# tataganesh/Query-Efficient-Approx-to-improve-OCR

Measured on AMD Instinct MI355X. Metric: patch-images/sec UNet->CRNN->CTC fwd+bwd, 32x128 grey, higher is better.
Workload: dtype f32 (GEMMs as scaled 2 x fp16 split products — three fp16 MFMAs per fp32 multiply-add — fp32 accumulate); 1 GPU; BASELINE configs[2]: full minibatch step of train_nn_area.py:212-287 — Phase A (UNet eval fwd, TopKCER k = 5 % of the minibatch, inner_limit = 4 jitter replicas fused in the batch dim, CRNN train-BN fwd+bwd, Adam(CRNN)) + Phase B (UNet train-BN -> CRNN BN-eval -> CTC mean + MSE -> backward -> Adam(UNet)) + greedy decode -> CER -> update_cer (:290-304) on synthetic POS-style 32x128 patches; batch_per_gpu=2048, global_batch=2048, full_step=True, crnn_wgrad=True, parallelism=dp1, hipgraph=False

## Files before the change

### query-efficient-approx-to-improve-ocr_amd/csrc/conv_wgrad.hip

```cpp
#include "common.h"
#include <type_traits>

namespace {

struct WgArgs {
  const float* p;
  const float* q;
  float* out;
  int B, PH, PW, QH, QW, R, C, KH, KW, pad_h, pad_w, stride_h, stride_w, ldp, ldq;
  int M, chunk, splits, accumulate;
  int r_tiles, c_tiles, tiles;
  long long slab;
  const float* pmax;
  const float* qmax;
};

constexpr int BKP_MAX = 32;

template <int P_LD, int Q_LD, int BKP>
struct WgGather {
  static constexpr int TPR = 256 / BKP;
  int grow, gl;
  int g_img, g_ph, g_pw;
  int qhw, dr, er, eq;
// ... 799 lines not shown
        *reinterpret_cast<bf16x4*>(Ps + 2 * P_PLANE + o) = l;
      }
    }
#pragma unroll
    for (int i = 0; i < NQ; ++i) {
      const int e = tid + 256 * i;
      const int c4 = e % CC4, hq = e / CC4;
      if (hq < HP) {
        const int o = row_off(hq, c4, CB);
        if constexpr (F16) {
          f16x4 h, l;
          qea_split2_f16(qreg[i], sq, h, l);
          *reinterpret_cast<f16x4*>(Qs + o) = h;
          *reinterpret_cast<f16x4*>(Qs + Q_PLANE + o) = l;
        } else {
          bf16x4 h, m, l;
          qea_split3(qreg[i], h, m, l);
          *reinterpret_cast<bf16x4*>(Qs + o) = h;
          *reinterpret_cast<bf16x4*>(Qs + Q_PLANE + o) = m;
          *reinterpret_cast<bf16x4*>(Qs + 2 * Q_PLANE + o) = l;
        }
      }
    }
  };
  const int g16 = lane >> 4, tq = (lane & 15) >> 2, tpp = lane & 3;
  const int l_pix = (g16 >> 1) * 8 + tq;
  const int l_ch = (g16 & 1) * 16 + tpp * 4;
  auto frag_p = [&](const __bf16* plane, int pix) -> frag_t {
    return __builtin_bit_cast(frag_t, RB == 64 ? tr_frag(plane + pix * 64 + (((wr ^ (pix >> 1)) & 1) << 5) + l_ch, 64) : tr_frag(plane + pix * 32 + l_ch, 32));
  };
  auto frag_q = [&](const __bf16* plane, int pix) -> frag_t {
    return __builtin_bit_cast(frag_t, CB == 64 ? tr_frag(plane + pix * 64 + (((wc ^ (pix >> 1)) & 1) << 5) + l_ch, 64) : tr_frag(plane + pix * 32 + l_ch, 32));
  };
  auto mma = [&](f32x16& a9, const frag_t* af, const frag_t* bf) {
    if constexpr (F16) {
      a9 = __builtin_amdgcn_mfma_f32_32x32x16_f16(af[1], bf[0], a9, 0, 0, 0);
      a9 = __builtin_amdgcn_mfma_f32_32x32x16_f16(af[0], bf[1], a9, 0, 0, 0);
      a9 = __builtin_amdgcn_mfma_f32_32x32x16_f16(af[0], bf[0], a9, 0, 0, 0);
    } else {
      a9 = __builtin_amdgcn_mfma_f32_32x32x16_bf16(af[2], bf[0], a9, 0, 0, 0);
      a9 = __builtin_amdgcn_mfma_f32_32x32x16_bf16(af[0], bf[2], a9, 0, 0, 0);
      a9 = __builtin_amdgcn_mfma_f32_32x32x16_bf16(af[1], bf[1], a9, 0, 0, 0);
      a9 = __builtin_amdgcn_mfma_f32_32x32x16_bf16(af[1], bf[0], a9, 0, 0, 0);
      a9 = __builtin_amdgcn_mfma_f32_32x32x16_bf16(af[0], bf[1], a9, 0, 0, 0);
      a9 = __builtin_amdgcn_mfma_f32_32x32x16_bf16(af[0], bf[0], a9, 0, 0, 0);
    }
  };

  int tile = split;
  if (tile < hp.n_tiles) fetch(tile);
  for (; tile < hp.n_tiles; tile += hp.splits) {
    __syncthreads();
    stage();
    __syncthreads();
    if (tile + hp.splits < hp.n_tiles) fetch(tile + hp.splits);
#pragma unroll 1
    for (int ks = wk; ks < 4; ks += WK) {
      const int py = (ks * 16) / SW, px0 = (ks * 16) % SW;
      frag_t af[NPL];
#pragma unroll
      for (int pl = 0; pl < NPL; ++pl) af[pl] = frag_p(Ps + pl * P_PLANE, ks * 16 + l_pix);
      if constexpr (RB == 32 || F16) {
        auto read_q = [&](int t, frag_t* bfr) {
          const int hq = (py + t / 3) * HW_ + px0 + t % 3 + l_pix;
#pragma unroll
          for (int pl = 0; pl < NPL; ++pl) bfr[pl] = frag_q(Qs + pl * Q_PLANE, hq);
        };
        frag_t bq2[2][NPL];
        read_q(0, bq2[0]);
#pragma unroll
        for (int t = 0; t < 9; ++t) {
          const frag_t* bf = bq2[t & 1];
          if (t + 1 < 9) read_q(t + 1, bq2[(t + 1) & 1]);
          mma(acc[t], af, bf);
          if (t + 1 < 9) {
            __builtin_amdgcn_sched_group_barrier(0x100, 2 * NPL, 0);
            __builtin_amdgcn_sched_group_barrier(0x008, F16 ? 3 : 6, 0);
          }
        }
      } else {
#pragma unroll
        for (int kh = 0; kh < 3; ++kh)
#pragma unroll
          for (int kw = 0; kw < 3; ++kw) {
            const int hq = (py + kh) * HW_ + px0 + kw + l_pix;
            frag_t bf[NPL];
#pragma unroll
            for (int pl = 0; pl < NPL; ++pl) bf[pl] = frag_q(Qs + pl * Q_PLANE, hq);
            mma(acc[kh * 3 + kw], af, bf);
          }
      }
    }
  }
  float* out = ws + ((size_t)split * WK + wk) * R * 9 * C;
  const int fr = lane & 31, fh = lane >> 5;
#pragma unroll
  for (int t = 0; t < 9; ++t)
#pragma unroll
    for (int r = 0; r < 16; ++r) {
      const int rr = r0 + wr * 32 + (r & 3) + 8 * (r >> 2) + 4 * fh;
      out[((size_t)rr * 9 + t) * C + c0 + wc * 32 + fr] = F16 ? (acc[t][r] * inv_p) * inv_q : acc[t][r];
    }
}

__device__ __forceinline__ f16x8 tr_pair128(const char* base) {
  typedef __attribute__((address_space(3))) s16x4* lds_ptr;
  const s16x4 lo = __builtin_amdgcn_ds_read_tr16_b64_v4i16((lds_ptr)(base));
  const s16x4 hi = __builtin_amdgcn_ds_read_tr16_b64_v4i16((lds_ptr)(base + 4 * 128));
  return __builtin_shufflevector(__builtin_bit_cast(f16x4, lo), __builtin_bit_cast(f16x4, hi), 0, 1, 2, 3, 4, 5, 6, 7);
}

__global__ void bias_finalize_kernel(const double* __restrict__ ws, int nblk, int R, float* __restrict__ out, int accumulate) {
  const int c = blockIdx.x * (blockDim.x >> 6) + (threadIdx.x >> 6);
  if (c >= R) return;
  const int lane = threadIdx.x & 63;
  double a = 0;
  for (int k = lane; k < nblk; k += 64) a += ws[(size_t)k * R + c];
  a = qea_wave_sum_d(a);
  if (lane == 0) out[c] = accumulate ? out[c] + (float)a : (float)a;
}

template <int SW>
constexpr size_t halo9_spec_lds() { return (size_t)2 * (2 * 64 * 64 * 2 + 2 * ((64 / SW + 2) * (SW + 2)) * 64 * 2); }

template <int SW>
__global__ __launch_bounds__(512) void wgrad_halo9_spec_kernel(const float* __restrict__ p, const float* __restrict__ q, float* __restrict__ ws, int B,
                                                               int H, int W, int R, int C, int ldp, int ldq, Halo9Plan hp,
                                                               const float* __restrict__ pmax, const float* __restrict__ qmax,
                                                               double* __restrict__ bias_ws) {
  constexpr int TH = 64 / SW, HWD = SW + 2, HH = TH + 2, HP = HH * HWD;
  constexpr int P_PLANE_B = 64 * 64 * 2, Q_PLANE_B = HP * 64 * 2;
  constexpr int BUF_B = 2 * P_PLANE_B + 2 * Q_PLANE_B;
  extern __shared__ __attribute__((aligned(16))) float smem[];
  char* lds = reinterpret_cast<char*>(smem);
  float sp, sq, inv_p, inv_q;
  qea_f16_scale(pmax[0], sp, inv_p);
  qea_f16_scale(qmax[0], sq, inv_q);
  const int tid = threadIdx.x, lane = tid & 63, wave = tid >> 6;
  int bid = qea_xcd_swizzle(blockIdx.x, gridDim.x);
  const int c_blk = bid % hp.c_blks;
  bid /= hp.c_blks;
  const int r_blk = bid % hp.r_blks;
  const int split = bid / hp.r_blks;
  const int r0 = r_blk * 64, c0 = c_blk * 64;
  const int ntl = (hp.n_tiles - split + hp.splits - 1) / hp.splits;

  if (wave >= 4) {
    const int pt = tid - 256;
    constexpr int NP = 64 * 16 / 256, NQ = (HP * 16 + 255) / 256;
    f32x4 preg[NP], qreg[NQ];
    const bool do_bias = bias_ws != nullptr && c_blk == 0;
    double bsum[4] = {0.0, 0.0, 0.0, 0.0};
    auto fetch = [&](int tile) {
      const int tx = tile % hp.tiles_x;
      const int ty = (tile / hp.tiles_x) % hp.tiles_y;
      const int b = tile / (hp.tiles_x * hp.tiles_y);
      const int x0 = tx * SW, y0 = ty * TH;
#pragma unroll
      for (int i = 0; i < NP; ++i) {
        const int e = pt + 256 * i;
        const int c4 = e % 16, pix = e / 16;
        const int py = pix / SW, px = pix - py * SW;
        preg[i] = *reinterpret_cast<const f32x4*>(p + ((size_t)(b * H + y0 + py) * W + x0 + px) * ldp + r0 + c4 * 4);
      }
#pragma unroll
      for (int i = 0; i < NQ; ++i) {
        const int e = pt + 256 * i;
        const int c4 = e % 16, hq = e / 16;
        f32x4 v = {0.f, 0.f, 0.f, 0.f};
        if (hq < HP) {
          const int hy = hq / HWD, hx = hq - hy * HWD;
          const int iy = y0 + hy - 1, ix = x0 + hx - 1;
          if ((unsigned)iy < (unsigned)H && (unsigned)ix < (unsigned)W) v = *reinterpret_cast<const f32x4*>(q + ((size_t)(b * H + iy) * W + ix) * ldq + c0 + c4 * 4);
        }
        qreg[i] = v;
      }
    };
    auto row_off = [](int pix, int c4) { return pix * 64 + ((((c4 >> 3) ^ (pix >> 1)) & 1) << 5) + (c4 & 7) * 4; };
    auto stage = [&](char* buf) {
      _Float16* Ps = reinterpret_cast<_Float16*>(buf);
      _Float16* Qs = reinterpret_cast<_Float16*>(buf + 2 * P_PLANE_B);
#pragma unroll
      for (int i = 0; i < NP; ++i) {
        const int e = pt + 256 * i;
        const int o = row_off(e / 16, e % 16);
        if (do_bias) {
#pragma unroll
          for (int k = 0; k < 4; ++k) bsum[k] += (double)preg[i][k];
        }
        f16x4 h, l;
        qea_split2_f16(preg[i], sp, h, l);
        *reinterpret_cast<f16x4*>(Ps + o) = h;
        *reinterpret_cast<f16x4*>(Ps + P_PLANE_B / 2 + o) = l;
      }
#pragma unroll
      for (int i = 0; i < NQ; ++i) {
        const int e = pt + 256 * i;
        const int hq = e / 16;
        if (hq < HP) {
          const int o = row_off(hq, e % 16);
          f16x4 h, l;
          qea_split2_f16(qreg[i], sq, h, l);
          *reinterpret_cast<f16x4*>(Qs + o) = h;
          *reinterpret_cast<f16x4*>(Qs + Q_PLANE_B / 2 + o) = l;
        }
      }
    };
    if (ntl > 0) {
      fetch(split);
      stage(lds);
      if (ntl > 1) fetch(split + hp.splits);
    }
    __syncthreads();
    for (int t = 0; t < ntl; ++t) {
      if (t + 1 < ntl) stage(lds + ((t + 1) & 1) * BUF_B);
      if (t + 2 < ntl) fetch(split + (t + 2) * hp.splits);
      __syncthreads();
    }
    if (do_bias) {
#pragma unroll
      for (int k = 0; k < 4; ++k) {
        double v = bsum[k];
        v += __shfl_xor(v, 16, 64);
        v += __shfl_xor(v, 32, 64);
        bsum[k] = v;
      }
      if (lane < 16) {
        double* dst = bias_ws + (size_t)(split * 4 + (wave - 4)) * R + r0 + lane * 4;
#pragma unroll
        for (int k = 0; k < 4; ++k) dst[k] = bsum[k];
      }
    }
    return;
  }

  const int wr = wave >> 1, wc = wave & 1;
  f32x16 acc[9];
#pragma unroll
  for (int t = 0; t < 9; ++t)
#pragma unroll
    for (int r = 0; r < 16; ++r) acc[t][r] = 0.f;
  const int g16 = lane >> 4, tq = (lane & 15) >> 2, tpp = lane & 3;
  const int l_pix = (g16 >> 1) * 8 + tq;
  const int l_ch = (g16 & 1) * 16 + tpp * 4;
  const int p_off = l_pix * 128 + ((((wr ^ (l_pix >> 1)) & 1) << 5) + l_ch) * 2;
  int TQ[2][2];
#pragma unroll
  for (int par = 0; par < 2; ++par)
#pragma unroll
    for (int b = 0; b < 2; ++b) {
      const int hs = (par ? (l_pix + 1) >> 1 : l_pix >> 1) + b;
      TQ[par][b] = l_pix * 128 + ((((wc ^ hs) & 1) << 5) + l_ch) * 2;
    }
  __syncthreads();
  for (int t = 0; t < ntl; ++t) {
    const char* buf = lds + (t & 1) * BUF_B;
    const char* Pb = buf + p_off;
    const char* Qb = buf + 2 * P_PLANE_B;
    auto read_p = [&](int ks, f16x8* af) {
      af[0] = tr_pair128(Pb + ks * 16 * 128);
      af[1] = tr_pair128(Pb + P_PLANE_B + ks * 16 * 128);
    };
    auto read_q = [&](int f, f16x8* bf) {
      const int ks = f / 9, tap = f % 9;
      const int py = (ks * 16) / SW, px0 = (ks * 16) % SW;
      const int c = (py + tap / 3) * HWD + px0 + tap % 3;
      const char* src = Qb + TQ[c & 1][(c >> 1) & 1] + c * 128;
      bf[0] = tr_pair128(src);
      bf[1] = tr_pair128(src + Q_PLANE_B);
    };
    f16x8 af[2][2], bq[2][2];
    read_p(0, af[0]);
    read_q(0, bq[0]);
#pragma unroll
    for (int f = 0; f < 36; ++f) {
      const int ks = f / 9, tap = f % 9;
      const f16x8* a = af[ks & 1];
      const f16x8* b = bq[f & 1];
      if (f + 1 < 36) read_q(f + 1, bq[(f + 1) & 1]);
      if (tap == 0 && ks + 1 < 4) read_p(ks + 1, af[(ks + 1) & 1]);
      acc[tap] = __builtin_amdgcn_mfma_f32_32x32x16_f16(a[1], b[0], acc[tap], 0, 0, 0);
      acc[tap] = __builtin_amdgcn_mfma_f32_32x32x16_f16(a[0], b[1], acc[tap], 0, 0, 0);
      acc[tap] = __builtin_amdgcn_mfma_f32_32x32x16_f16(a[0], b[0], acc[tap], 0, 0, 0);
      if (f + 1 < 36) {
        if (tap == 0 && ks + 1 < 4) __builtin_amdgcn_sched_group_barrier(0x100, 8, 0);
        else __builtin_amdgcn_sched_group_barrier(0x100, 4, 0);
        __builtin_amdgcn_sched_group_barrier(0x008, 3, 0);
      }
    }
    __syncthreads();
  }
  float* out = ws + (size_t)split * R * 9 * C;
  const int fr = lane & 31, fh = lane >> 5;
#pragma unroll
  for (int t = 0; t < 9; ++t)
#pragma unroll
    for (int r = 0; r < 16; ++r) {
      const int rr = r0 + wr * 32 + (r & 3) + 8 * (r >> 2) + 4 * fh;
      out[((size_t)rr * 9 + t) * C + c0 + wc * 32 + fr] = (acc[t][r] * inv_p) * inv_q;
    }
}

constexpr int H9R_ROWS = 8, H9R_HWD = 34;
constexpr size_t halo9_ring_lds() { return (size_t)2 * (2 * 64 * 64 * 2) + (size_t)2 * H9R_ROWS * H9R_HWD * 64 * 2; }

__global__ __launch_bounds__(512) void wgrad_halo9_ring_kernel(const float* __restrict__ p, const float* __restrict__ q, float* __restrict__ ws, int B, int H,
                                                               int W, int R, int C, int ldp, int ldq, Halo9Plan hp, const float* __restrict__ pmax,
                                                               const float* __restrict__ qmax, double* __restrict__ bias_ws) {
  constexpr int SW = 32, TH = 2, HWD = H9R_HWD;
  constexpr int P_PLANE_B = 64 * 64 * 2, QR_PLANE_B = H9R_ROWS * HWD * 64 * 2;
  extern __shared__ __attribute__((aligned(16))) float smem[];
  char* const Pbase = reinterpret_cast<char*>(smem);
  char* const Qbase = Pbase + 2 * (2 * P_PLANE_B);
  float sp, sq, inv_p, inv_q;
  qea_f16_scale(pmax[0], sp, inv_p);
  qea_f16_scale(qmax[0], sq, inv_q);
  const int tid = threadIdx.x, lane = tid & 63, wave = tid >> 6;
  int bid = qea_xcd_swizzle(blockIdx.x, gridDim.x);
  const int c_blk = bid % hp.c_blks;
  bid /= hp.c_blks;
  const int r_blk = bid % hp.r_blks;
  const int split = bid / hp.r_blks;
  const int r0 = r_blk * 64, c0 = c_blk * 64;
  const int n_strips = B * hp.tiles_x;
  const int s0 = (int)((long long)n_strips * split / hp.splits), s1 = (int)((long long)n_strips * (split + 1) / hp.splits);
  const int ntl = (s1 - s0) * hp.tiles_y;
  auto ring_of = [&](int t) { return ((t + t / hp.tiles_y) * 2) & 7; };

  if (wave >= 4) {
    const int pt = tid - 256;
    constexpr int NP = 64 * 16 / 256, NQ = (4 * HWD * 16 + 255) / 256;
    f32x4 preg[NP], qreg[NQ];
    int q_rows = 0, q_ring0 = 0;
    const bool do_bias = bias_ws != nullptr && c_blk == 0;
    double bsum[4] = {0.0, 0.0, 0.0, 0.0};
    auto fetch = [&](int t) {
      const int st = s0 + t / hp.tiles_y, ty = t % hp.tiles_y;
      const int b = st / hp.tiles_x, x0 = (st % hp.tiles_x) * SW, y0 = ty * TH;
#pragma unroll
      for (int i = 0; i < NP; ++i) {
        const int e = pt + 256 * i;
        const int c4 = e % 16, pix = e / 16;
        const int py = pix / SW, px = pix - py * SW;
        preg[i] = *reinterpret_cast<const f32x4*>(p + ((size_t)(b * H + y0 + py) * W + x0 + px) * ldp + r0 + c4 * 4);
      }
      const int hy0 = ty == 0 ? 0 : 2;
      q_rows = 4 - hy0;
      q_ring0 = (ring_of(t) + hy0) & 7;
#pragma unroll
      for (int i = 0; i < NQ; ++i) {
        const int e = pt + 256 * i;
        const int c4 = e % 16, hq = e / 16;
        f32x4 v = {0.f, 0.f, 0.f, 0.f};
        if (hq < q_rows * HWD) {
          const int hy = hy0 + hq / HWD, hx = hq % HWD;
          const int iy = y0 + hy - 1, ix = x0 + hx - 1;
          if ((unsigned)iy < (unsigned)H && (unsigned)ix < (unsigned)W) v = *reinterpret_cast<const f32x4*>(q + ((size_t)(b * H + iy) * W + ix) * ldq + c0 + c4 * 4);
        }
        qreg[i] = v;
      }
    };
    auto row_off = [](int pix, int c4) { return pix * 64 + ((((c4 >> 3) ^ (pix >> 1)) & 1) << 5) + (c4 & 7) * 4; };
    auto stage = [&](int pbuf) {
      _Float16* Ps = reinterpret_cast<_Float16*>(Pbase + pbuf * (2 * P_PLANE_B));
      _Float16* Qs = reinterpret_cast<_Float16*>(Qbase);
#pragma unroll
      for (int i = 0; i < NP; ++i) {
        const int e = pt + 256 * i;
        const int o = row_off(e / 16, e % 16);
        if (do_bias) {
#pragma unroll
          for (int k = 0; k < 4; ++k) bsum[k] += (double)preg[i][k];
        }
        f16x4 h, l;
        qea_split2_f16(preg[i], sp, h, l);
        *reinterpret_cast<f16x4*>(Ps + o) = h;
        *reinterpret_cast<f16x4*>(Ps + P_PLANE_B / 2 + o) = l;
      }
#pragma unroll
      for (int i = 0; i < NQ; ++i) {
        const int e = pt + 256 * i;
        const int hq = e / 16;
        if (hq < q_rows * HWD) {
          const int rr = (q_ring0 + hq / HWD) & 7;
          const int o = row_off(rr * HWD + hq % HWD, e % 16);
          f16x4 h, l;
          qea_split2_f16(qreg[i], sq, h, l);
          *reinterpret_cast<f16x4*>(Qs + o) = h;
          *reinterpret_cast<f16x4*>(Qs + QR_PLANE_B / 2 + o) = l;
        }
      }
    };
    if (ntl > 0) {
      fetch(0);
      stage(0);
      if (ntl > 1) fetch(1);
    }
    __syncthreads();
    for (int t = 0; t < ntl; ++t) {
      if (t + 1 < ntl) stage((t + 1) & 1);
      if (t + 2 < ntl) fetch(t + 2);
      __syncthreads();
    }
    if (do_bias) {
#pragma unroll
      for (int k = 0; k < 4; ++k) {
        double v = bsum[k];
        v += __shfl_xor(v, 16, 64);
        v += __shfl_xor(v, 32, 64);
        bsum[k] = v;
      }
      if (lane < 16) {
        double* dst = bias_ws + (size_t)(split * 4 + (wave - 4)) * R + r0 + lane * 4;
#pragma unroll
        for (int k = 0; k < 4; ++k) dst[k] = bsum[k];
      }
    }
    return;
  }

  const int wr = wave >> 1, wc = wave & 1;
  f32x16 acc[9];
#pragma unroll
  for (int t = 0; t < 9; ++t)
#pragma unroll
    for (int r = 0; r < 16; ++r) acc[t][r] = 0.f;
  const int g16 = lane >> 4, tq = (lane & 15) >> 2, tpp = lane & 3;
  const int l_pix = (g16 >> 1) * 8 + tq;
  const int l_ch = (g16 & 1) * 16 + tpp * 4;
  const int p_off = l_pix * 128 + ((((wr ^ (l_pix >> 1)) & 1) << 5) + l_ch) * 2;
  int TQ[2][2];
#pragma unroll
  for (int par = 0; par < 2; ++par)
#pragma unroll
    for (int b = 0; b < 2; ++b) {
      const int hs = (par ? (l_pix + 1) >> 1 : l_pix >> 1) + b;
      TQ[par][b] = l_pix * 128 + ((((wc ^ hs) & 1) << 5) + l_ch) * 2;
    }
  __syncthreads();
  for (int t = 0; t < ntl; ++t) {
    const char* Pb = Pbase + (t & 1) * (2 * P_PLANE_B) + p_off;
    const int g = ring_of(t);
    int QB[4][2][2];
#pragma unroll
    for (int k = 0; k < 4; ++k) {
      const int rowoff = ((g + k) & 7) * (HWD * 128);
#pragma unroll
      for (int par = 0; par < 2; ++par)
#pragma unroll
        for (int bb = 0; bb < 2; ++bb) QB[k][par][bb] = TQ[par][bb] + rowoff;
    }
    auto read_p = [&](int ks, f16x8* af) {
      af[0] = tr_pair128(Pb + ks * 16 * 128);
      af[1] = tr_pair128(Pb + P_PLANE_B + ks * 16 * 128);
    };
    auto read_q = [&](int f, f16x8* bf) {
      const int ks = f / 9, tap = f % 9;
      const int py = (ks * 16) / SW, px0 = (ks * 16) % SW;
      const int k = py + tap / 3, col = px0 + tap % 3;
      const char* src = Qbase + QB[k][col & 1][((col >> 1) + k) & 1] + col * 128;
      bf[0] = tr_pair128(src);
      bf[1] = tr_pair128(src + QR_PLANE_B);
    };
    f16x8 af[2][2], bq[2][2];
    read_p(0, af[0]);
    read_q(0, bq[0]);
#pragma unroll
    for (int f = 0; f < 36; ++f) {
      const int ks = f / 9, tap = f % 9;
      const f16x8* a = af[ks & 1];
      const f16x8* b = bq[f & 1];
      if (f + 1 < 36) read_q(f + 1, bq[(f + 1) & 1]);
      if (tap == 0 && ks + 1 < 4) read_p(ks + 1, af[(ks + 1) & 1]);
      acc[tap] = __builtin_amdgcn_mfma_f32_32x32x16_f16(a[1], b[0], acc[tap], 0, 0, 0);
      acc[tap] = __builtin_amdgcn_mfma_f32_32x32x16_f16(a[0], b[1], acc[tap], 0, 0, 0);
      acc[tap] = __builtin_amdgcn_mfma_f32_32x32x16_f16(a[0], b[0], acc[tap], 0, 0, 0);
      if (f + 1 < 36) {
        if (tap == 0 && ks + 1 < 4) __builtin_amdgcn_sched_group_barrier(0x100, 8, 0);
        else __builtin_amdgcn_sched_group_barrier(0x100, 4, 0);
        __builtin_amdgcn_sched_group_barrier(0x008, 3, 0);
      }
    }
    __syncthreads();
  }
  float* out = ws + (size_t)split * R * 9 * C;
  const int fr = lane & 31, fh = lane >> 5;
#pragma unroll
  for (int t = 0; t < 9; ++t)
#pragma unroll
    for (int r = 0; r < 16; ++r) {
      const int rr = r0 + wr * 32 + (r & 3) + 8 * (r >> 2) + 4 * fh;
      out[((size_t)rr * 9 + t) * C + c0 + wc * 32 + fr] = (acc[t][r] * inv_p) * inv_q;
    }
}

Halo9Plan halo9_plan(const qea_wgrad_desc* d) {
  Halo9Plan h = {false, 0, 0, 0, 0, 0, 0, 0, 0, 64, 64, 1, 0};
  if (d->KH != 3 || d->KW != 3 || d->pad_h != 1 || d->pad_w != 1 || d->stride_h != 1 || d->stride_w != 1 || d->PH != d->QH || d->PW != d->QW) return h;
  if (d->R % 32 || d->C % 32) return h;
  h.sw = (d->PW % 32 == 0) ? 32 : (d->PW == 16 ? 16 : 0);
  if (!h.sw) return h;
  h.th = 64 / h.sw;
  if (d->PH % h.th) return h;
  h.tiles_x = d->PW / h.sw;
  h.tiles_y = d->PH / h.th;
  const long long nt = (long long)d->B * h.tiles_x * h.tiles_y;
  if (nt > 0x7fffffffLL) return h;
  h.n_tiles = (int)nt;
  h.rb = h.cb = (d->R % 64 || d->C % 64) ? 32 : 64;
  h.wk = 4 / ((h.rb / 32) * (h.cb / 32));
  h.r_blks = d->R / h.rb;
  h.c_blks = d->C / h.cb;
  h.spec = (h.rb == 64 && d->p_absmax && d->q_absmax && d->tile != 29) ? 1 : 0;
  int splits = d->splits > 0 ? d->splits : (h.spec ? 256 : 512) / (h.r_blks * h.c_blks);
  if (splits > h.n_tiles / 8) splits = h.n_tiles / 8;
  if (h.spec && h.sw == 32 && splits > d->B * h.tiles_x) splits = d->B * h.tiles_x;
  if (splits < 1) splits = 1;
  h.splits = splits;
  h.ok = true;
  return h;
}

template <int SW, int RB, int CB, int NPL>
int launch_halo9_(const qea_wgrad_desc* d, const Halo9Plan& h, hipStream_t s) {
  constexpr size_t lds = (size_t)NPL * (64 * RB + H9_HP_MAX * CB) * 2;
  const int rc = reserve_lds<wgrad_halo9_bf3_kernel<SW, RB, CB, NPL>>("qea_conv_wgrad", lds);
  if (rc != QEA_OK) return rc;
  hipLaunchKernelGGL((wgrad_halo9_bf3_kernel<SW, RB, CB, NPL>), dim3((unsigned)((long long)h.r_blks * h.c_blks * h.splits)), dim3(256), lds, s, d->p, d->q,
                     (float*)d->workspace, d->B, d->PH, d->PW, d->R, d->C, d->ldp, d->ldq, h, d->p_absmax, d->q_absmax);
  return QEA_OK;
}

template <int SW, int RB, int CB>
int launch_halo9_any(const qea_wgrad_desc* d, const Halo9Plan& h, hipStream_t s) {
  return (d->p_absmax && d->q_absmax) ? launch_halo9_<SW, RB, CB, 2>(d, h, s) : launch_halo9_<SW, RB, CB, 3>(d, h, s);
}

template <auto Kernel, size_t LDS>
int launch_halo9_pc(const qea_wgrad_desc* d, const Halo9Plan& h, hipStream_t s, double* bias_ws) {
  const int rc = reserve_lds<Kernel>("qea_conv_wgrad", LDS);
  if (rc != QEA_OK) return rc;
  hipLaunchKernelGGL(Kernel, dim3((unsigned)((long long)h.r_blks * h.c_blks * h.splits)), dim3(512), LDS, s, d->p, d->q, (float*)d->workspace, d->B, d->PH, d->PW,
                     d->R, d->C, d->ldp, d->ldq, h, d->p_absmax, d->q_absmax, bias_ws);
  return QEA_OK;
}

int launch_halo9(const qea_wgrad_desc* d, const Halo9Plan& h, hipStream_t s, double* bias_ws) {
  if (h.spec)
    return h.sw == 32 ? launch_halo9_pc<wgrad_halo9_ring_kernel, halo9_ring_lds()>(d, h, s, bias_ws)
                      : launch_halo9_pc<wgrad_halo9_spec_kernel<16>, halo9_spec_lds<16>()>(d, h, s, bias_ws);
  if (h.sw == 32) return h.rb == 64 ? launch_halo9_any<32, 64, 64>(d, h, s) : launch_halo9_any<32, 32, 32>(d, h, s);
  return h.rb == 64 ? launch_halo9_any<16, 64, 64>(d, h, s) : launch_halo9_any<16, 32, 32>(d, h, s);
}

enum Family { GENERIC, HALO_F32, NINE_TAP };

struct Route {
  Family family;
  union {
    Plan generic;
    HaloPlan halo;
    Halo9Plan nine;
  };
  size_t slab_floats;
  int n_slabs;
  size_t slab_bytes;
  size_t bias_bytes;
  size_t workspace_bytes;
  bool fuses_bias;
  bool wants_absmax;
  int split_tag;
  const char* error;
};

Route route(const qea_wgrad_desc* d) {
  Route r = {};
  const int tile = d->tile;
  const int both_tag = (d->p_absmax && d->q_absmax) ? 2 : 1;
  r.slab_floats = (size_t)d->R * d->KH * d->KW * d->C;
  if ((tile == 0 && qea_split_bf16_enabled()) || tile == 23 || tile == 29) {
    r.nine = halo9_plan(d);
    if (r.nine.ok) {
      r.family = NINE_TAP;
      r.n_slabs = r.nine.splits * r.nine.wk;
      r.fuses_bias = r.nine.spec;
      if (r.nine.spec && d->dbias) r.bias_bytes = (size_t)r.nine.splits * 4 * d->R * sizeof(double);
      r.wants_absmax = true;
      r.split_tag = both_tag;
    } else if (tile != 0) {
      r.error = "qea_conv_wgrad: tile 23 (nine-tap split-bf16) needs a 3x3 pad-1 stride-1 conv, R,C multiples of 64, PW in {16, 32k}";
    }
  }
  if (r.family == GENERIC && !r.error && (tile == 0 || tile == 6)) {
    r.halo = halo_plan(d);
    if (r.halo.ok) {
      r.family = HALO_F32;
      r.n_slabs = r.halo.grid * r.halo.wk;
    } else if (tile != 0) {
      r.error = "qea_conv_wgrad: tile 6 (LDS-halo) needs a 3x3 pad-1 stride-1 conv with R,C in {32,64}, PW %% 32 == 0";
    }
  }
  if (r.family == GENERIC && !r.error) {
    const Tile* t = find_tile(tile ? tile : auto_tile(d->R, d->C));
    if (!t) {
      r.error = "qea_conv_wgrad: unknown tile %d";
      return r;
    }
    r.generic = make_plan(d, t);
    r.n_slabs = r.generic.splits > 1 ? r.generic.splits : 0;
    r.wants_absmax = t->id >= FIRST_SPLIT_TILE;
    r.split_tag = r.wants_absmax ? both_tag : 0;
  }
  r.slab_bytes = r.n_slabs ? slab_workspace_bytes(r.slab_floats, r.n_slabs) : 0;
  r.workspace_bytes = r.slab_bytes + r.bias_bytes;
  return r;
}

bool has_dims(const qea_wgrad_desc* d) { return d && d->R > 0 && d->C > 0 && d->B > 0; }

}

extern "C" int qea_conv_wgrad_fuses_bias(const qea_wgrad_desc* d) { return (has_dims(d) && route(d).fuses_bias) ? 1 : 0; }

extern "C" int qea_conv_wgrad_wants_absmax(const qea_wgrad_desc* d) { return (has_dims(d) && route(d).wants_absmax) ? 1 : 0; }

extern "C" size_t qea_conv_wgrad_workspace_bytes(const qea_wgrad_desc* d) { return has_dims(d) ? route(d).workspace_bytes : 0; }

extern "C" int qea_conv_wgrad(const qea_wgrad_desc* d, void* stream) {
  int rc = validate(d, "qea_conv_wgrad");
  if (rc != QEA_OK) return rc;
  const Route r = route(d);
  QEA_REQUIRE(!r.error, r.error, d->tile);
  const size_t need = r.slab_bytes + r.bias_bytes;
  QEA_REQUIRE(need == 0 || (d->workspace && d->workspace_bytes >= need && ((uintptr_t)d->workspace & 15) == 0),
              "qea_conv_wgrad: workspace of %zu bytes required, %zu given", need, (size_t)d->workspace_bytes);
  QEA_REQUIRE(!d->dbias || r.bias_bytes, "qea_conv_wgrad: dbias is taken by the producer / consumer nine-tap form only (ask qea_conv_wgrad_fuses_bias first)");
  hipStream_t s = (hipStream_t)stream;
  qea_prof_begin(QEA_PROF_CONV_WGRAD, s);
  double* bias_ws = r.bias_bytes ? reinterpret_cast<double*>(reinterpret_cast<char*>(d->workspace) + r.slab_bytes) : nullptr;
  switch (r.family) {
    case HALO_F32: rc = launch_halo(d, r.halo, s); break;
    case NINE_TAP: rc = launch_halo9(d, r.nine, s, bias_ws); break;
    case GENERIC: rc = launch_generic(d, r.generic, r.n_slabs, s); break;
  }
  if (rc != QEA_OK) {
    qea_prof_abort(QEA_PROF_CONV_WGRAD);
    return rc;
  }
  if (r.n_slabs) reduce_slabs((float*)d->workspace, d->dw, (long long)r.slab_floats / 4, r.n_slabs, d->accumulate, s);
  if (bias_ws)
    hipLaunchKernelGGL(bias_finalize_kernel, dim3(qea_cdiv(d->R, 4)), dim3(256), 0, s, (const double*)bias_ws, r.nine.splits * 4, d->R, d->dbias, d->accumulate);
  const double M = (double)d->B * d->PH * d->PW;
  qea_prof_end(QEA_PROF_CONV_WGRAD, s, 2.0 * M * (double)r.slab_floats, 4.0 * (M * d->R + (double)d->B * d->QH * d->QW * d->C + (double)r.slab_floats),
               r.split_tag);
  QEA_CHECK_LAUNCH();
  return QEA_OK;
}
```

Measured before the change: 21430 patch-images/s.

## Generalize ring wgrad kernel to 32/64 channel blocks with tap-split waves

Templates the producer/consumer ring 3x3 weight-gradient kernel on row and column channel block sizes (32 or 64), so layers whose channel counts are not multiples of 64 also use it instead of the older generic halo path. When a block has fewer than four 32x32 sub-blocks, the four consumer waves split the nine taps among themselves rather than each owning a sub-block. The planner now picks row and column blocks independently and sizes splits for the new occupancy. The trade-off is more template instantiations, an uneven tap split across waves, and a changed split heuristic.

Result: no change. 21660 patch-images/s, median of 6 (+1.1%).

```diff
diff --git a/query-efficient-approx-to-improve-ocr_amd/csrc/conv_wgrad.hip b/query-efficient-approx-to-improve-ocr_amd/csrc/conv_wgrad.hip
--- a/query-efficient-approx-to-improve-ocr_amd/csrc/conv_wgrad.hip
+++ b/query-efficient-approx-to-improve-ocr_amd/csrc/conv_wgrad.hip
@@ -1125,13 +1125,27 @@
 }
 
 constexpr int H9R_ROWS = 8, H9R_HWD = 34;
-constexpr size_t halo9_ring_lds() { return (size_t)2 * (2 * 64 * 64 * 2) + (size_t)2 * H9R_ROWS * H9R_HWD * 64 * 2; }
-
-__global__ __launch_bounds__(512) void wgrad_halo9_ring_kernel(const float* __restrict__ p, const float* __restrict__ q, float* __restrict__ ws, int B, int H,
-                                                               int W, int R, int C, int ldp, int ldq, Halo9Plan hp, const float* __restrict__ pmax,
-                                                               const float* __restrict__ qmax, double* __restrict__ bias_ws) {
+template <int RB, int CB>
+constexpr size_t halo9_ring_lds() { return (size_t)2 * (2 * 64 * RB * 2) + (size_t)2 * H9R_ROWS * H9R_HWD * CB * 2; }
+
+template <int ROWB>
+__device__ __forceinline__ f16x8 tr_pair(const char* base) {
+  typedef __attribute__((address_space(3))) s16x4* lds_ptr;
+  const s16x4 lo = __builtin_amdgcn_ds_read_tr16_b64_v4i16((lds_ptr)(base));
+  const s16x4 hi = __builtin_amdgcn_ds_read_tr16_b64_v4i16((lds_ptr)(base + 4 * ROWB));
+  return __builtin_shufflevector(__builtin_bit_cast(f16x4, lo), __builtin_bit_cast(f16x4, hi), 0, 1, 2, 3, 4, 5, 6, 7);
+}
+
+template <int RB, int CB>
+__global__ __launch_bounds__(512)
+void wgrad_halo9_ring_kernel(const float* __restrict__ p, const float* __restrict__ q, float* __restrict__ ws, int B, int H, int W, int R, int C, int ldp,
+                             int ldq, Halo9Plan hp, const float* __restrict__ pmax, const float* __restrict__ qmax, double* __restrict__ bias_ws) {
   constexpr int SW = 32, TH = 2, HWD = H9R_HWD;
-  constexpr int P_PLANE_B = 64 * 64 * 2, QR_PLANE_B = H9R_ROWS * HWD * 64 * 2;
+  constexpr int PROW_B = RB * 2, QROW_B = CB * 2;
+  constexpr int P_PLANE_B = 64 * PROW_B, QR_PLANE_B = H9R_ROWS * HWD * QROW_B;
+  constexpr int RC4 = RB / 4, CC4 = CB / 4;
+  constexpr int NSB = (RB / 32) * (CB / 32), TW = 4 / NSB, NT = (9 + TW - 1) / TW;
+  static_assert((RB == 32 || RB == 64) && (CB == 32 || CB == 64), "channel blocks of 32 or 64");
   extern __shared__ __attribute__((aligned(16))) float smem[];
   char* const Pbase = reinterpret_cast<char*>(smem);
   char* const Qbase = Pbase + 2 * (2 * P_PLANE_B);
@@ -1144,7 +1158,7 @@
   bid /= hp.c_blks;
   const int r_blk = bid % hp.r_blks;
   const int split = bid / hp.r_blks;
-  const int r0 = r_blk * 64, c0 = c_blk * 64;
+  const int r0 = r_blk * RB, c0 = c_blk * CB;
   const int n_strips = B * hp.tiles_x;
   const int s0 = (int)((long long)n_strips * split / hp.splits), s1 = (int)((long long)n_strips * (split + 1) / hp.splits);
   const int ntl = (s1 - s0) * hp.tiles_y;
@@ -1152,7 +1166,7 @@
 
   if (wave >= 4) {
     const int pt = tid - 256;
-    constexpr int NP = 64 * 16 / 256, NQ = (4 * HWD * 16 + 255) / 256;
+    constexpr int NP = 64 * RC4 / 256, NQ = (4 * HWD * CC4 + 255) / 256;
     f32x4 preg[NP], qreg[NQ];
     int q_rows = 0, q_ring0 = 0;
     const bool do_bias = bias_ws != nullptr && c_blk == 0;
@@ -1163,7 +1177,7 @@
 #pragma unroll
       for (int i = 0; i < NP; ++i) {
         const int e = pt + 256 * i;
-        const int c4 = e % 16, pix = e / 16;
+        const int c4 = e % RC4, pix = e / RC4;
         const int py = pix / SW, px = pix - py * SW;
         preg[i] = *reinterpret_cast<const f32x4*>(p + ((size_t)(b * H + y0 + py) * W + x0 + px) * ldp + r0 + c4 * 4);
       }
@@ -1173,7 +1187,7 @@
 #pragma unroll
       for (int i = 0; i < NQ; ++i) {
         const int e = pt + 256 * i;
-        const int c4 = e % 16, hq = e / 16;
+        const int c4 = e % CC4, hq = e / CC4;
         f32x4 v = {0.f, 0.f, 0.f, 0.f};
         if (hq < q_rows * HWD) {
           const int hy = hy0 + hq / HWD, hx = hq % HWD;
@@ -1183,14 +1197,14 @@
         qreg[i] = v;
       }
     };
-    auto row_off = [](int pix, int c4) { return pix * 64 + ((((c4 >> 3) ^ (pix >> 1)) & 1) << 5) + (c4 & 7) * 4; };
+    auto row_off = [](int pix, int c4, int ch) { return ch == 64 ? pix * 64 + ((((c4 >> 3) ^ (pix >> 1)) & 1) << 5) + (c4 & 7) * 4 : pix * 32 + c4 * 4; };
     auto stage = [&](int pbuf) {
       _Float16* Ps = reinterpret_cast<_Float16*>(Pbase + pbuf * (2 * P_PLANE_B));
       _Float16* Qs = reinterpret_cast<_Float16*>(Qbase);
 #pragma unroll
       for (int i = 0; i < NP; ++i) {
         const int e = pt + 256 * i;
-        const int o = row_off(e / 16, e % 16);
+        const int o = row_off(e / RC4, e % RC4, RB);
         if (do_bias) {
 #pragma unroll
           for (int k = 0; k < 4; ++k) bsum[k] += (double)preg[i][k];
@@ -1203,10 +1217,10 @@
 #pragma unroll
       for (int i = 0; i < NQ; ++i) {
         const int e = pt + 256 * i;
-        const int hq = e / 16;
+        const int hq = e / CC4;
         if (hq < q_rows * HWD) {
           const int rr = (q_ring0 + hq / HWD) & 7;
-          const int o = row_off(rr * HWD + hq % HWD, e % 16);
+          const int o = row_off(rr * HWD + hq % HWD, e % CC4, CB);
           f16x4 h, l;
           qea_split2_f16(qreg[i], sq, h, l);
           *reinterpret_cast<f16x4*>(Qs + o) = h;
@@ -1229,11 +1243,12 @@
 #pragma unroll
       for (int k = 0; k < 4; ++k) {
         double v = bsum[k];
+        if constexpr (RC4 == 8) v += __shfl_xor(v, 8, 64);
         v += __shfl_xor(v, 16, 64);
         v += __shfl_xor(v, 32, 64);
         bsum[k] = v;
       }
-      if (lane < 16) {
+      if (lane < RC4) {
         double* dst = bias_ws + (size_t)(split * 4 + (wave - 4)) * R + r0 + lane * 4;
 #pragma unroll
         for (int k = 0; k < 4; ++k) dst[k] = bsum[k];
@@ -1242,6 +1257,7 @@
     return;
   }
 
+  if constexpr (NSB == 4) {
   const int wr = wave >> 1, wc = wave & 1;
   f32x16 acc[9];
 #pragma unroll
@@ -1315,6 +1331,100 @@
       const int rr = r0 + wr * 32 + (r & 3) + 8 * (r >> 2) + 4 * fh;
       out[((size_t)rr * 9 + t) * C + c0 + wc * 32 + fr] = (acc[t][r] * inv_p) * inv_q;
     }
+  } else {
+  const int sb = wave % NSB;
+  const int tg = __builtin_amdgcn_readfirstlane(wave / NSB);
+  const int wr = RB == 64 ? sb : 0, wc = CB == 64 ? sb : 0;
+  f32x16 acc[NT];
+#pragma unroll
+  for (int t = 0; t < NT; ++t)
+#pragma unroll
+    for (int r = 0; r < 16; ++r) acc[t][r] = 0.f;
+  const int g16 = lane >> 4, tq = (lane & 15) >> 2, tpp = lane & 3;
+  const int l_pix = (g16 >> 1) * 8 + tq;
+  const int l_ch = (g16 & 1) * 16 + tpp * 4;
+  const int p_off = RB == 64 ? l_pix * 128 + ((((wr ^ (l_pix >> 1)) & 1) << 5) + l_ch) * 2 : l_pix * 64 + l_ch * 2;
+  int TQ[2][2];
+#pragma unroll
+  for (int par = 0; par < 2; ++par)
+#pragma unroll
+    for (int b = 0; b < 2; ++b) {
+      const int hs = (par ? (l_pix + 1) >> 1 : l_pix >> 1) + b;
+      TQ[par][b] = CB == 64 ? l_pix * 128 + ((((wc ^ hs) & 1) << 5) + l_ch) * 2 : l_pix * 64 + l_ch * 2;
+    }
+  auto tiles = [&](auto tgc) {
+    constexpr int TG = decltype(tgc)::value;
+    constexpr int NTG = (9 - TG + TW - 1) / TW, NF = 4 * NTG;
+    for (int t = 0; t < ntl; ++t) {
+      const char* Pb = Pbase + (t & 1) * (2 * P_PLANE_B) + p_off;
+      const int g = ring_of(t);
+      int QB[4][2][2];
+#pragma unroll
+      for (int k = 0; k < 4; ++k) {
+        const int rowoff = ((g + k) & 7) * (HWD * QROW_B);
+#pragma unroll
+        for (int par = 0; par < 2; ++par)
+#pragma unroll
+          for (int bb = 0; bb < 2; ++bb) QB[k][par][bb] = TQ[par][bb] + rowoff;
+      }
+      auto read_p = [&](int ks, f16x8* af) {
+        af[0] = tr_pair<PROW_B>(Pb + ks * 16 * PROW_B);
+        af[1] = tr_pair<PROW_B>(Pb + P_PLANE_B + ks * 16 * PROW_B);
+      };
+      auto read_q = [&](int f, f16x8* bf) {
+        const int ks = f / NTG, tap = TG + TW * (f % NTG);
+        const int py = (ks * 16) / SW, px0 = (ks * 16) % SW;
+        const int k = py + tap / 3, col = px0 + tap % 3;
+        const char* src = Qbase + (CB == 64 ? QB[k][col & 1][((col >> 1) + k) & 1] : QB[k][0][0]) + col * QROW_B;
+        bf[0] = tr_pair<QROW_B>(src);
+        bf[1] = tr_pair<QROW_B>(src + QR_PLANE_B);
+      };
+      f16x8 af[2][2], bq[2][2];
+      read_p(0, af[0]);
+      read_q(0, bq[0]);
+#pragma unroll
+      for (int f = 0; f < NF; ++f) {
+        const int ks = f / NTG, j = f % NTG;
+        const f16x8* a = af[ks & 1];
+        const f16x8* b = bq[f & 1];
+        if (f + 1 < NF) read_q(f + 1, bq[(f + 1) & 1]);
+        if (j == 0 && ks + 1 < 4) read_p(ks + 1, af[(ks + 1) & 1]);
+        acc[j] = __builtin_amdgcn_mfma_f32_32x32x16_f16(a[1], b[0], acc[j], 0, 0, 0);
+        acc[j] = __builtin_amdgcn_mfma_f32_32x32x16_f16(a[0], b[1], acc[j], 0, 0, 0);
+        acc[j] = __builtin_amdgcn_mfma_f32_32x32x16_f16(a[0], b[0], acc[j], 0, 0, 0);
+        if (f + 1 < NF) {
+          if (j == 0 && ks + 1 < 4) __builtin_amdgcn_sched_group_barrier(0x100, 8, 0);
+          else __builtin_amdgcn_sched_group_barrier(0x100, 4, 0);
+          __builtin_amdgcn_sched_group_barrier(0x008, 3, 0);
+        }
+      }
+      __syncthreads();
+    }
+  };
+  __syncthreads();
+  if constexpr (TW == 2) {
+    if (tg == 0) tiles(std::integral_constant<int, 0>{});
+    else tiles(std::integral_constant<int, 1>{});
+  } else {
+    if (tg == 0) tiles(std::integral_constant<int, 0>{});
+    else if (tg == 1) tiles(std::integral_constant<int, 1>{});
+    else if (tg == 2) tiles(std::integral_constant<int, 2>{});
+    else tiles(std::integral_constant<int, 3>{});
+  }
+  float* out = ws + (size_t)split * R * 9 * C;
+  const int fr = lane & 31, fh = lane >> 5;
+#pragma unroll
+  for (int j = 0; j < NT; ++j) {
+    const int tap = tg + TW * j;
+    if (tap < 9) {
+#pragma unroll
+      for (int r = 0; r < 16; ++r) {
+        const int rr = r0 + wr * 32 + (r & 3) + 8 * (r >> 2) + 4 * fh;
+        out[((size_t)rr * 9 + tap) * C + c0 + wc * 32 + fr] = (acc[j][r] * inv_p) * inv_q;
+      }
+    }
+  }
+  }
 }
 
 Halo9Plan halo9_plan(const qea_wgrad_desc* d) {
@@ -1330,14 +1440,23 @@
   const long long nt = (long long)d->B * h.tiles_x * h.tiles_y;
   if (nt > 0x7fffffffLL) return h;
   h.n_tiles = (int)nt;
-  h.rb = h.cb = (d->R % 64 || d->C % 64) ? 32 : 64;
-  h.wk = 4 / ((h.rb / 32) * (h.cb / 32));
+  const bool pc = d->p_absmax && d->q_absmax && d->tile != 29;
+  if (pc && h.sw == 32) {
+    h.rb = d->R % 64 ? 32 : 64;
+    h.cb = d->C % 64 ? 32 : 64;
+    h.spec = 1;
+  } else {
+    h.rb = h.cb = (d->R % 64 || d->C % 64) ? 32 : 64;
+    h.spec = (pc && h.rb == 64) ? 1 : 0;
+  }
+  h.wk = h.spec ? 1 : 4 / ((h.rb / 32) * (h.cb / 32));
   h.r_blks = d->R / h.rb;
   h.c_blks = d->C / h.cb;
-  h.spec = (h.rb == 64 && d->p_absmax && d->q_absmax && d->tile != 29) ? 1 : 0;
-  int splits = d->splits > 0 ? d->splits : (h.spec ? 256 : 512) / (h.r_blks * h.c_blks);
-  if (splits > h.n_tiles / 8) splits = h.n_tiles / 8;
-  if (h.spec && h.sw == 32 && splits > d->B * h.tiles_x) splits = d->B * h.tiles_x;
+  const int resident = (!h.spec || (h.sw == 32 && h.cb == 32)) ? 512 : 256;
+  int splits = d->splits > 0 ? d->splits : resident / (h.r_blks * h.c_blks);
+  const bool ring = h.spec && h.sw == 32;
+  if (splits > h.n_tiles / 8 && !(ring && d->splits > 0)) splits = h.n_tiles / 8;
+  if (ring && splits > d->B * h.tiles_x) splits = d->B * h.tiles_x;
   if (splits < 1) splits = 1;
   h.splits = splits;
   h.ok = true;
@@ -1369,9 +1488,13 @@
 }
 
 int launch_halo9(const qea_wgrad_desc* d, const Halo9Plan& h, hipStream_t s, double* bias_ws) {
-  if (h.spec)
-    return h.sw == 32 ? launch_halo9_pc<wgrad_halo9_ring_kernel, halo9_ring_lds()>(d, h, s, bias_ws)
-                      : launch_halo9_pc<wgrad_halo9_spec_kernel<16>, halo9_spec_lds<16>()>(d, h, s, bias_ws);
+  if (h.spec && h.sw == 32) {
+    if (h.rb == 64 && h.cb == 64) return launch_halo9_pc<wgrad_halo9_ring_kernel<64, 64>, halo9_ring_lds<64, 64>()>(d, h, s, bias_ws);
+    if (h.rb == 64) return launch_halo9_pc<wgrad_halo9_ring_kernel<64, 32>, halo9_ring_lds<64, 32>()>(d, h, s, bias_ws);
+    if (h.cb == 64) return launch_halo9_pc<wgrad_halo9_ring_kernel<32, 64>, halo9_ring_lds<32, 64>()>(d, h, s, bias_ws);
+    return launch_halo9_pc<wgrad_halo9_ring_kernel<32, 32>, halo9_ring_lds<32, 32>()>(d, h, s, bias_ws);
+  }
+  if (h.spec) return launch_halo9_pc<wgrad_halo9_spec_kernel<16>, halo9_spec_lds<16>()>(d, h, s, bias_ws);
   if (h.sw == 32) return h.rb == 64 ? launch_halo9_any<32, 64, 64>(d, h, s) : launch_halo9_any<32, 32, 32>(d, h, s);
   return h.rb == 64 ? launch_halo9_any<16, 64, 64>(d, h, s) : launch_halo9_any<16, 32, 32>(d, h, s);
 }
```
